# fractalclockwork/CS267_HW3

Measured on NVIDIA B200. Metric: kmers_per_s_insert_plus_traverse, higher is better.
Workload: dtype u128

## Files before the change

cs267_hw3_b200/csrc/ctable.cuh:

```cuda
#pragma once
#include "kernels.cuh"

namespace kh {

#ifndef KH_CT_BUCKETS2
#define KH_CT_BUCKETS2 2176
#endif
#ifndef KH_CT_THREADS
#define KH_CT_THREADS 512
#endif
#ifndef KH_CT_MINBLOCKS
#define KH_CT_MINBLOCKS 2
#endif
#ifndef KH_CT_JUMPS
#define KH_CT_JUMPS 3
#endif
template <int W> struct CtBuild {
    static constexpr u32 kMaxBuckets = (W == 1) ? 1536u : (u32)KH_CT_BUCKETS2;
    static constexpr u32 kMaxSlots = kMaxBuckets * (u32)Slot<W>::kPerBucket;
    static constexpr u32 kOffSucc = kMaxBuckets * 32u;
    static constexpr u32 kOffPd = kOffSucc + kMaxSlots * 2u;
    static constexpr u32 kOffOff = kOffPd + kMaxSlots * 4u;
    static constexpr u32 kOffCode = kOffOff + kMaxSlots * 2u;
    static constexpr u32 kSmem = kOffCode + kMaxSlots;
// ... 280 lines not shown
    }
}

__global__ void ct_mark_filed_kernel(const u32* __restrict__ xin_cnt, u32* __restrict__ xin_done, const u32* __restrict__ extra_cnt,
                                     u32* __restrict__ extra_done, const CtCaps caps, int world) {
    const int s = (int)threadIdx.x;
    if (s < world) xin_done[s] = min(xin_cnt[s], caps.xin_cap);
    if (s == 0) *extra_done = min(*extra_cnt, caps.extra_cap);
}

__global__ void __launch_bounds__(1024)
ct_layout_kernel(const u32* __restrict__ chunk_cursor, u32 nchunks, const CtGeom g, const CtCaps caps, u32 per_bucket, u32 max_slots,
                 u32* __restrict__ chunk_base, u32* __restrict__ pool_off, Counters* ctr) {
    __shared__ u64 s_warp[33];
    constexpr u32 kPer = 8;
    u64 carry_b = 0, carry_p = 0;
    for (u32 c0 = 0; c0 < nchunks; c0 += blockDim.x * kPer) {
        const u32 first = c0 + threadIdx.x * kPer;
        u32 capb[kPer], chars[kPer];
        u64 sum_b = 0, sum_p = 0;
#pragma unroll
        for (u32 q = 0; q < kPer; ++q) {
            const u32 c = first + q;
            capb[q] = 0; chars[q] = 0;
            if (c < nchunks) {
                const u32 load = min(chunk_cursor[c], max_slots);
                if (load) {
                    const u64 want_slots = ((u64)load * g.lf_inv_q16 + 65535u) >> 16;
                    capb[q] = (u32)min((u64)g.max_buckets, max((want_slots + per_bucket - 1) / per_bucket, (u64)(load / per_bucket + 1)));
                }
                chars[q] = (load + 15u) & ~15u;
            }
            sum_b += capb[q]; sum_p += chars[q];
        }
        u64 tot_b, tot_p;
        u64 eb = carry_b + block_exclusive_scan(sum_b, s_warp, tot_b);
        u64 ep = carry_p + block_exclusive_scan(sum_p, s_warp, tot_p);
#pragma unroll
        for (u32 q = 0; q < kPer; ++q) {
            const u32 c = first + q;
            if (c < nchunks) { chunk_base[c] = (u32)eb; pool_off[c] = (u32)ep; }
            eb += capb[q]; ep += chars[q];
        }
        carry_b += tot_b; carry_p += tot_p;
    }
    if (threadIdx.x == 0) {
        chunk_base[nchunks] = (u32)carry_b;
        pool_off[nchunks] = (u32)carry_p;
        if (carry_b > caps.nbuckets_alloc || carry_p > caps.pool_cap) atomicOr(&ctr->errors, kErrTableFull);
    }
}

template <int W> __device__ __forceinline__ u32 ct_tag(typename Slot<W>::value_t v);
template <> __device__ __forceinline__ u32 ct_tag<1>(u64 v) { return (u32)(v >> 6); }
template <> __device__ __forceinline__ u32 ct_tag<2>(u128 v) { return (u32)(v.lo >> 6); }

template <int W, bool VOLATILE>
__device__ __forceinline__ void ct_lds_tags(unsigned saddr, u64 (&w)[4]) {
    if (W == 1) {
        if (VOLATILE) {
            asm volatile("ld.volatile.shared.v2.u64 {%0,%1}, [%2];" : "=l"(w[0]), "=l"(w[1]) : "r"(saddr) : "memory");
            asm volatile("ld.volatile.shared.v2.u64 {%0,%1}, [%2+16];" : "=l"(w[2]), "=l"(w[3]) : "r"(saddr) : "memory");
        } else {
            asm volatile("ld.shared.v2.u64 {%0,%1}, [%2];" : "=l"(w[0]), "=l"(w[1]) : "r"(saddr));
            asm volatile("ld.shared.v2.u64 {%0,%1}, [%2+16];" : "=l"(w[2]), "=l"(w[3]) : "r"(saddr));
        }
    } else {
        if (VOLATILE) {
            asm volatile("ld.volatile.shared.u64 %0, [%1];" : "=l"(w[0]) : "r"(saddr) : "memory");
            asm volatile("ld.volatile.shared.u64 %0, [%1+16];" : "=l"(w[1]) : "r"(saddr) : "memory");
        } else {
            asm volatile("ld.shared.u64 %0, [%1];" : "=l"(w[0]) : "r"(saddr));
            asm volatile("ld.shared.u64 %0, [%1+16];" : "=l"(w[1]) : "r"(saddr));
        }
    }
}
__device__ __forceinline__ u64 ct_lds64(unsigned saddr) {
    u64 x;
    asm volatile("ld.volatile.shared.u64 %0, [%1];" : "=l"(x) : "r"(saddr) : "memory");
    return x;
}
template <int W> __device__ __forceinline__ bool ct_verify(unsigned saddr, int i, u64 low, typename Slot<W>::value_t key, u64& idx_word);
template <> __device__ __forceinline__ bool ct_verify<1>(unsigned, int, u64 low, u64 key, u64& idx_word) {
    idx_word = low;
    return CtSlot<1>::same_key(low, key);
}
template <> __device__ __forceinline__ bool ct_verify<2>(unsigned saddr, int i, u64 low, u128 key, u64& idx_word) {
    idx_word = ct_lds64(saddr + 16u * i + 8u);
    return (((idx_word ^ key.hi) << kIdxBits) | ((low ^ key.lo) >> 6)) == 0ull;
}

template <int W>
__device__ __forceinline__ int ct_smem_insert(typename Slot<W>::value_t* s_tab, unsigned s_base, u32 nb, typename Slot<W>::value_t val) {
    typedef Slot<W> S;
    typedef typename S::value_t V;
    const u32 tag = ct_tag<W>(val);
    u32 b = ct_bucket_in_chunk(CtSlot<W>::hash32(val), nb);
    for (u32 tries = 0; tries < nb;) {
        u64 w[4];
        ct_lds_tags<W, true>(s_base + b * 32u, w);
        int j = -1;
        u32 match = 0;
#pragma unroll
        for (int i = S::kPerBucket - 1; i >= 0; --i) {
            const bool e = ((u32)w[i] & 7u) == 0u;
            j = e ? i : j;
            match |= (!e && (u32)(w[i] >> 6) == tag) ? (1u << i) : 0u;
        }
        if (match) {
#pragma unroll
            for (int i = 0; i < S::kPerBucket; ++i) {
                u64 iw;
                if ((match >> i) & 1u) if (ct_verify<W>(s_base + b * 32u, i, w[i], val, iw)) return -1;
            }
        }
        if (j < 0) { b = (b + 1 == nb) ? 0u : b + 1; ++tries; continue; }
        const V old = S::cas_shared(s_tab + b * S::kPerBucket + j, S::zero(), val);
        if (S::empty(old)) return (int)(b * S::kPerBucket + j);
        if (CtSlot<W>::same_key(old, val)) return -1;
    }
    return -2;
}

constexpr int kFindMiss = -1, kFindNext = -2;
template <int W>
__device__ __forceinline__ void ct_lds_bucket(unsigned saddr, u64 (&q)[4]) {
    asm volatile("ld.shared.v2.u64 {%0,%1}, [%2];" : "=l"(q[0]), "=l"(q[1]) : "r"(saddr));
    asm volatile("ld.shared.v2.u64 {%0,%1}, [%2+16];" : "=l"(q[2]), "=l"(q[3]) : "r"(saddr));
}
template <int W> __device__ __forceinline__ int ct_find_step(unsigned saddr, typename Slot<W>::value_t key);
template <> __device__ __forceinline__ int ct_find_step<1>(unsigned saddr, u64 key) {
    u64 q[4];
    ct_lds_bucket<1>(saddr, q);
    int res = kFindNext;
#pragma unroll
    for (int i = 3; i >= 0; --i) {
        const bool e = ((u32)q[i] & 7u) == 0u;
        const bool m = (((q[i] ^ key) << kIdxBits) >> (kIdxBits + 6)) == 0ull;
        res = e ? kFindMiss : (m ? (int)(q[i] >> (64 - kIdxBits)) - 1 : res);
    }
    return res;
}
template <> __device__ __forceinline__ int ct_find_step<2>(unsigned saddr, u128 key) {
    u64 q[4];
    ct_lds_bucket<2>(saddr, q);
    int res = kFindNext;
#pragma unroll
    for (int i = 1; i >= 0; --i) {
        const bool e = ((u32)q[2 * i] & 7u) == 0u;
        const bool m = (((q[2 * i + 1] ^ key.hi) << kIdxBits) | ((q[2 * i] ^ key.lo) >> 6)) == 0ull;
        res = e ? kFindMiss : (m ? (int)(q[2 * i + 1] >> (64 - kIdxBits)) - 1 : res);
    }
    return res;
}

template <int W>
__global__ void __launch_bounds__(kCtBuildThreads, KH_CT_MINBLOCKS)
ct_build_kernel(const typename Slot<W>::value_t* __restrict__ fine, const u32* __restrict__ chunk_cursor,
                const u32* __restrict__ chunk_base, const u32* __restrict__ pool_off,
                typename Slot<W>::value_t* __restrict__ table, u32* __restrict__ seg_base,
                u64* __restrict__ link, u64* __restrict__ meta, typename Slot<W>::value_t* __restrict__ ext_key,
                unsigned char* __restrict__ pool, const CtGeom g, const CtCaps caps, Counters* ctr) {
    typedef Slot<W> S;
    typedef CtSlot<W> CS;
    typedef typename S::value_t V;
    typedef CtBuild<W> B;
    extern __shared__ __align__(128) unsigned char s_bld[];
    unsigned char* const s_raw = s_bld;
    V* s_tab = reinterpret_cast<V*>(s_raw);
    unsigned short* s_succ = reinterpret_cast<unsigned short*>(s_raw + B::kOffSucc);
    unsigned char* s_pool = s_raw + B::kOffSucc;
    u32* s_pd = reinterpret_cast<u32*>(s_raw + B::kOffPd);
    unsigned short* s_off = reinterpret_cast<unsigned short*>(s_raw + B::kOffOff);
    unsigned char* s_code = s_raw + B::kOffCode;
    __shared__ u32 s_inserted, s_dups, s_nheads, s_seg0, s_chars, s_err;
    const u32 c = blockIdx.x;
    const u32 b0 = chunk_base[c], nb = chunk_base[c + 1] - b0;
    const u32 cnt = min(chunk_cursor[c], B::kMaxSlots);
    if (nb == 0) {
        if (threadIdx.x == 0) seg_base[c] = 0;
        return;
    }
    const unsigned s_base = (unsigned)__cvta_generic_to_shared(s_tab);
    const int k = g.k;
    constexpr int kBatch = 4;
    V v[kBatch];
#pragma unroll
    for (int r = 0; r < kBatch; ++r) {
        const u32 i = threadIdx.x + r * kCtBuildThreads;
        v[r] = i < cnt ? fine[ct_fine_index<W>(c, i, g.chunks_per_rank)] : S::zero();
    }
    if (threadIdx.x == 0) { s_inserted = 0; s_dups = 0; s_nheads = 0; s_chars = 0; s_err = 0; }
    {
        uint4* s4 = reinterpret_cast<uint4*>(s_raw);
        for (u32 i = threadIdx.x; i < nb * 2u; i += kCtBuildThreads) s4[i] = make_uint4(0, 0, 0, 0);
        for (u32 i = threadIdx.x; i < cnt; i += kCtBuildThreads) s_pd[i] = (kPredNone << 16) | 1u;
    }
    __syncthreads();
    u32 inserted = 0, dups = 0, err = 0;
    for (u32 base = 0; base < cnt; base += kCtBuildThreads * kBatch) {
        V nxt[kBatch];
#pragma unroll
        for (int r = 0; r < kBatch; ++r) {
            const u32 i = base + kCtBuildThreads * kBatch + threadIdx.x + r * kCtBuildThreads;
            nxt[r] = i < cnt ? fine[ct_fine_index<W>(c, i, g.chunks_per_rank)] : S::zero();
        }
#pragma unroll
        for (int r = 0; r < kBatch; ++r) {
            const u32 node = base + threadIdx.x + r * kCtBuildThreads;
            if (node >= cnt) continue;
            const int slot = ct_smem_insert<W>(s_tab, s_base, nb, CS::with_idx(v[r], node + 1u));
            inserted += (slot >= 0);
            dups += (slot == -1);
            if (slot == -2) err |= kErrTableFull;
            s_succ[node] = (unsigned short)(slot >= 0 ? (u32)slot : kSuccDead);
        }
#pragma unroll
        for (int r = 0; r < kBatch; ++r) v[r] = nxt[r];
    }
    inserted = __reduce_add_sync(kFullMask, inserted);
    dups = __reduce_add_sync(kFullMask, dups);
    err = __reduce_or_sync(kFullMask, err);
    if (lane_id() == 0) {
        if (inserted) atomicAdd(&s_inserted, inserted);
        if (dups) atomicAdd(&s_dups, dups);
        if (err) atomicOr(&s_err, err);
    }
    __syncthreads();
#pragma unroll 1
    for (u32 base = threadIdx.x; base < cnt; base += 2 * kCtBuildThreads) {
        u32 slot[2], b[2], code[2];
        V key[2];
        int res[2];
#pragma unroll
        for (int q = 0; q < 2; ++q) {
            const u32 node = base + q * kCtBuildThreads;
            slot[q] = node < cnt ? (u32)s_succ[node] : kSuccDead;
        }
#pragma unroll
        for (int q = 0; q < 2; ++q) {
            const V cur = slot[q] != kSuccDead ? s_tab[slot[q]] : S::zero();
            const u32 f = slot[q] != kSuccDead ? S::fwd(cur) : kExtF;
            code[q] = f | ((slot[q] != kSuccDead && S::back(cur) == kExtF) ? kCodeBackF : 0u);
            key[q] = S::next_key(CS::strip(cur), k);
            b[q] = ct_bucket_in_chunk(CS::hash32(key[q]), nb);
        }
#pragma unroll
        for (int q = 0; q < 2; ++q) res[q] = (code[q] & 7u) != kExtF ? ct_find_step<W>(s_base + b[q] * 32u, key[q]) : kFindMiss;
#pragma unroll
        for (int q = 0; q < 2; ++q) {
            for (u32 tries = 1; res[q] == kFindNext && tries < nb; ++tries) {
                b[q] = (b[q] + 1 == nb) ? 0u : b[q] + 1;
                res[q] = ct_find_step<W>(s_base + b[q] * 32u, key[q]);
            }
        }
#pragma unroll
        for (int q = 0; q < 2; ++q) {
            const u32 node = base + q * kCtBuildThreads;
            if (node >= cnt) continue;
            s_code[node] = (unsigned char)code[q];
            u32 sc = slot[q] == kSuccDead ? kSuccDead : kSuccTail;
            if ((code[q] & 7u) != kExtF) {
                if (res[q] < 0) {
                    sc = kSuccExt | slot[q];
                } else {
                    sc = (u32)res[q];
                    s_pd[res[q]] = (node << 16) | 1u;
                }
            }
            s_succ[node] = (unsigned short)sc;
        }
    }
    __syncthreads();
#pragma unroll 1
    for (u32 node = threadIdx.x; node < cnt; node += kCtBuildThreads) {
        const u32 s = s_succ[node];
        if (s < kSuccExt && (s_pd[s] >> 16) != node) s_code[s] |= (unsigned char)kCodeMulti;
    }
    __syncthreads();
    for (u32 base = 0; base < cnt; base += kCtBuildThreads) {
        const u32 node = base + threadIdx.x;
        bool head = false, dead = true;
        if (node < cnt) {
            dead = s_succ[node] == kSuccDead;
            head = !dead && ((s_pd[node] >> 16) == kPredNone || (s_code[node] & (kCodeBackF | kCodeMulti)));
        }
        const u32 bal = __ballot_sync(kFullMask, head);
        u32 first = 0;
        if (lane_id() == 0 && bal) first = atomicAdd(&s_nheads, (u32)__popc(bal));
        first = __shfl_sync(kFullMask, first, 0);
        if (head) s_pd[node] = (node << 16) | (first + __popc(bal & ((1u << lane_id()) - 1u)));
        else if (dead && node < cnt) s_pd[node] = node << 16;
    }
    __syncthreads();
    const u32 nheads = s_nheads;
    if (threadIdx.x == 0) {
        u32 seg0 = nheads ? atomicAdd(&ctr->next_seg, nheads) : 0u;
        if (seg0 + nheads > caps.seg_cap) { ct_internal(ctr, kSiteSegCap); seg0 = caps.seg_cap; }
        s_seg0 = seg0;
        seg_base[c] = seg0;
    }
    u32 active = 0;
#pragma unroll 1
    for (u32 i = 0, node = threadIdx.x; node < cnt; ++i, node += kCtBuildThreads) {
        const u32 pd = s_pd[node];
        active |= ((pd >> 16) != node) ? (1u << i) : 0u;
    }
    for (int round = 0; round < (14 + KH_CT_JUMPS - 1) / KH_CT_JUMPS; ++round) {
#pragma unroll 1
        for (int rep = 0; rep < KH_CT_JUMPS; ++rep) {
#pragma unroll 1
            for (u32 m = active; m; m &= m - 1u) {
                const u32 i = (u32)__ffs((int)m) - 1u, node = threadIdx.x + i * kCtBuildThreads;
                const u32 pd = s_pd[node], a = pd >> 16;
                const u32 pa = s_pd[a], a2 = pa >> 16;
                if (a2 == a) { active &= ~(1u << i); continue; }
                s_pd[node] = (a2 << 16) | ((pd + pa) & 0xFFFFu);
            }
        }
        if (!__syncthreads_or(active != 0u)) break;
    }
    __syncthreads();
    const u32 seg0 = s_seg0;
    const u32 my_bits = (u32)g.rank << kRankShift;
    const u64 pool0 = pool_off[c];
    if (seg0 < caps.seg_cap) {
    #pragma unroll 1
    for (u32 node = threadIdx.x; node < cnt; node += kCtBuildThreads) {
            const u32 s = s_succ[node];
            if (s == kSuccDead) continue;
            const u32 pd = s_pd[node], a = pd >> 16;
            const bool root = a == node;
            const u32 pa = root ? pd : s_pd[a];
            if ((pa >> 16) != a) continue;
            const u32 f = s_code[node] & 7u;
            bool last = f == kExtF || s >= kSuccExt;
            u32 next_hi = f == kExtF ? kLinkTail : kLinkPending;
            if (!last) {
                const u32 ps = s_pd[s];
                if ((ps >> 16) == s) { last = true; next_hi = my_bits | (seg0 + (ps & 0xFFFFu)); }
            }
            if (!last) continue;
            const u32 n = (root ? 0u : (pd & 0xFFFFu)) + (f != kExtF ? 1u : 0u);
            const u32 off = atomicAdd(&s_chars, n);
            s_off[a] = (unsigned short)off;
            const u32 gseg = seg0 + (pa & 0xFFFFu);
            link[gseg] = ((u64)next_hi << 32) | (next_hi == kLinkTail ? 0u : n);
            meta[gseg] = ((pool0 + off) << 24) | n;
            if (next_hi == kLinkPending) ext_key[gseg] = S::next_key(CS::strip(s_tab[s & 0x7FFFu]), k);
        }
    }
    __syncthreads();
#pragma unroll 1
    for (u32 node = threadIdx.x; node < cnt; node += kCtBuildThreads) {
        const u32 code = s_code[node];
        if ((code & 7u) == kExtF) continue;
        const u32 pd = s_pd[node], a = pd >> 16;
        const bool root = a == node;
        if (!root && (s_pd[a] >> 16) != a) continue;
        s_pool[(u32)s_off[a] + (root ? 0u : (pd & 0xFFFFu))] = ext_char(code & 7u);
    }
    {
        const u32 nslots = nb * S::kPerBucket;
        for (u32 i = threadIdx.x; i < nslots; i += kCtBuildThreads) {
            const V cur = s_tab[i];
            if (S::empty(cur)) continue;
            const u32 node = CS::idx(cur) - 1u, pd = s_pd[node];
            s_tab[i] = CS::with_idx(cur, (pd >> 16) == node ? (pd & 0xFFFFu) + 1u : 0u);
        }
    }
    asm volatile("fence.proxy.async.shared::cta;" ::: "memory");
    __syncthreads();
    {
        const u32 tab_bytes = nb * 32u, pool_bytes = (s_chars + 15u) & ~15u;
        constexpr u32 kPiece = 8192u;
        const u32 tab_pieces = (tab_bytes + kPiece - 1u) / kPiece, pool_pieces = (pool_bytes + kPiece - 1u) / kPiece;
        if (lane_id() == 0) {
            unsigned char* g_tab = reinterpret_cast<unsigned char*>(table + (u64)b0 * S::kPerBucket);
            bool any = false;
            for (u32 pc = threadIdx.x >> 5; pc < tab_pieces + pool_pieces; pc += kCtBuildThreads / 32) {
                const bool is_tab = pc < tab_pieces;
                const u32 o = (is_tab ? pc : pc - tab_pieces) * kPiece;
                const u32 bytes = min(kPiece, (is_tab ? tab_bytes : pool_bytes) - o);
                const unsigned src = (unsigned)__cvta_generic_to_shared(is_tab ? s_raw + o : s_pool + o);
                unsigned char* dst = is_tab ? g_tab + o : pool + pool0 + o;
                asm volatile("cp.async.bulk.global.shared::cta.bulk_group [%0], [%1], %2;" ::"l"(dst), "r"(src), "r"(bytes) : "memory");
                any = true;
            }
            if (any) {
                asm volatile("cp.async.bulk.commit_group;" ::: "memory");
                asm volatile("cp.async.bulk.wait_group.read 0;" ::: "memory");
            }
        }
    }
    if (threadIdx.x == 0) {
        if (s_inserted) atomicAdd(&ctr->n_inserted, (u64)s_inserted);
        if (s_dups) atomicAdd(&ctr->n_duplicates, (u64)s_dups);
        if (s_err) atomicOr(&ctr->errors, s_err);
    }
}

template <int W>
__device__ __forceinline__ bool ct_lookup_chunk(const typename Slot<W>::value_t* __restrict__ table, const u32* __restrict__ chunk_base,
                                                u32 chunk, typename Slot<W>::value_t key, typename Slot<W>::value_t& found) {
    typedef Slot<W> S;
    typedef typename S::value_t V;
    const u32 b0 = chunk_base[chunk], nb = chunk_base[chunk + 1] - b0;
    if (nb == 0) return false;
    u32 b = ct_bucket_in_chunk(CtSlot<W>::hash32(key), nb);
    for (u32 tries = 0; tries < nb; ++tries) {
        u64 q[4];
        load256_nc(table + (u64)(b0 + b) * S::kPerBucket, q);
        bool hole = false, hit = false;
#pragma unroll
        for (int i = 0; i < S::kPerBucket; ++i) {
            const V cur = S::from_bucket(q, i);
            const bool e = S::empty(cur);
            if (!hole && !hit && !e && CtSlot<W>::same_key(cur, key)) { found = cur; hit = true; }
            hole = hole || e;
        }
        if (hit) return true;
        if (hole) return false;
        b = (b + 1 == nb) ? 0u : b + 1;
    }
    return false;
}
// ... 445 lines not shown
```

cs267_hw3_b200/csrc/slot.cuh:

```cuda
#pragma once
#include <cstdint>
#include <cuda_runtime.h>

namespace kh {

typedef unsigned long long u64;
typedef unsigned int u32;

constexpr u32 kExtF = 4;
constexpr u32 kExtBad = 7;

struct alignas(16) u128 {
    u64 lo, hi;
};

constexpr u64 ext_lut_entry(u64 lut, int idx, u64 code) { return (lut & ~(7ull << (3 * idx))) | (code << (3 * idx)); }
constexpr u64 kExtLut = ext_lut_entry(ext_lut_entry(ext_lut_entry(ext_lut_entry(ext_lut_entry(
                            0x7FFFFFFFFFFFFFFFull, 1, 0), 3, 1), 6, 4), 7, 2), 20, 3);
__host__ __device__ __forceinline__ u32 ext_code(unsigned char c) {
    const u32 i = c & 31u;
    const bool letter = (c & 0xE0u) == 0x40u && i <= 20u;
    return letter ? ((u32)(kExtLut >> (3u * i)) & 7u) : kExtBad;
}
#ifdef __CUDACC__
// ... 246 lines not shown


__host__ __device__ __forceinline__ int minimizer_len(int k) {
    return k <= 14 ? k : (k <= 18 ? 11 : (k <= 29 ? 13 : (k <= 40 ? 21 : 31)));
}
__host__ __device__ __forceinline__ u32 mmer_order(u64 x) {
    return (u32)((x * 0x9E3779B97F4A7C15ull) >> 32);
}
template <int W> __host__ __device__ __forceinline__ u64 minimizer_value(typename Slot<W>::value_t v, int k, int m);
template <> __host__ __device__ __forceinline__ u64 minimizer_value<1>(u64 v, int k, int m) {
    const u64 key = v >> 6, mask = (m >= 32) ? ~0ull : ((1ull << (2 * m)) - 1ull);
    u32 best = 0xFFFFFFFFu;
    u64 bx = 0;
    for (int s = 2 * (k - m); s >= 0; s -= 2) {
        const u64 x = (key >> s) & mask;
        const u32 g = mmer_order(x);
        if (g < best) { best = g; bx = x; }
    }
    return bx;
}
template <> __host__ __device__ __forceinline__ u64 minimizer_value<2>(u128 v, int k, int m) {
    const u64 lo = (v.lo >> 6) | (v.hi << 58), hi = v.hi >> 6, mask = (m >= 32) ? ~0ull : ((1ull << (2 * m)) - 1ull);
    u32 best = 0xFFFFFFFFu;
    u64 bx = 0;
    for (int s = 2 * (k - m); s >= 0; s -= 2) {
        const u64 x = (s >= 64 ? (hi >> (s - 64)) : (s == 0 ? lo : ((lo >> s) | (hi << (64 - s))))) & mask;
        const u32 g = mmer_order(x);
        if (g < best) { best = g; bx = x; }
    }
    return bx;
}
__host__ __device__ __forceinline__ int owner_minimizer_len(int k) { return k <= 14 ? k : 7; }

template <int W> __host__ __device__ __forceinline__ u64 owner_hash_of(typename Slot<W>::value_t v, int k, int m) {
    return m ? fmix64(minimizer_value<W>(v, k, m) + 0x632BE59BD9B4E019ull) : Slot<W>::owner_hash(v);
}

__host__ __device__ __forceinline__ u64 bucket_of(u64 h, u64 nbuckets) {
#ifdef __CUDA_ARCH__
    return __umul64hi(h, nbuckets);
#else
    return (u64)(((unsigned __int128)h * nbuckets) >> 64);
#endif
}

template <int W>
__host__ __device__ __forceinline__ u32 owner_of(typename Slot<W>::value_t v, int world, int k, int m) {
    return (u32)bucket_of(owner_hash_of<W>(v, k, m), (u64)world);
}

template <int W> struct RegionOf { static constexpr u64 kBuckets = (W == 1) ? 4 : 16; };
template <int W>
__host__ __device__ __forceinline__ u64 place_bucket_from(u64 minimizer_hash, typename Slot<W>::value_t v, u64 nbuckets) {
    constexpr u64 G = RegionOf<W>::kBuckets;
    const u64 region = bucket_of(fmix64(minimizer_hash ^ 0x9E3779B97F4A7C15ull), nbuckets / G);
    return region * G + (Slot<W>::hash(v) & (G - 1));
}
template <int W>
__host__ __device__ __forceinline__ u64 place_bucket(typename Slot<W>::value_t v, int k, int m, u64 nbuckets) {
    if (m == 0) return bucket_of(Slot<W>::hash(v), nbuckets);
    return place_bucket_from<W>(fmix64(minimizer_value<W>(v, k, m) + 0x632BE59BD9B4E019ull), v, nbuckets);
}

constexpr u32 kIdxBits = 14;
constexpr u32 kMinMul = 0x9E3779B1u;
constexpr u32 kMinAdd = 0x7F4A7C15u;

__host__ __device__ __forceinline__ int ct_minimizer_len(int k) { return k >= 31 ? 15 : (k >= 23 ? 13 : (k >= 17 ? k - 6 : k)); }
__host__ __device__ __forceinline__ int ct_window(int k) { const int w = k - ct_minimizer_len(k) + 1; return w > 32 ? 32 : w; }
__host__ __device__ __forceinline__ bool ct_supported(int k) { return k >= 17 && k <= 54; }
__host__ __device__ __forceinline__ int ct_slot_words(int k) { return (2 * k + 6 + (int)kIdxBits <= 64) ? 1 : 2; }

__host__ __device__ __forceinline__ u32 ct_funnel_r(u32 lo, u32 hi, u32 s) {
#ifdef __CUDA_ARCH__
    return __funnelshift_r(lo, hi, s);
#else
    return s ? ((lo >> s) | (hi << (32 - s))) : lo;
#endif
}
__host__ __device__ __forceinline__ u32 ct_mulhi32(u32 a, u32 b) {
#ifdef __CUDA_ARCH__
    return __umulhi(a, b);
#else
    return (u32)(((u64)a * b) >> 32);
#endif
}
__host__ __device__ __forceinline__ u32 ct_min_hash_words(u32 a, u32 b, u32 c, u32 d, int m, int win) {
    const u32 mul = kMinMul << (32 - 2 * m);
    u32 best = 0xFFFFFFFFu;
    int rem = win;
    for (int it = 0; it < 2; ++it) {
        if (rem >= 16) {
#pragma unroll
            for (int j = 0; j < 16; ++j) {
                const u32 h = ct_funnel_r(a, b, 2u * j) * mul + kMinAdd;
                best = h < best ? h : best;
            }
        } else {
#pragma unroll
            for (int j = 0; j < 16; ++j) {
                u32 h = ct_funnel_r(a, b, 2u * j) * mul + kMinAdd;
                h = (j < rem) ? h : 0xFFFFFFFFu;
                best = h < best ? h : best;
            }
        }
        if (rem <= 16) break;
        rem -= 16; a = b; b = c; c = d; d = 0;
    }
    return best;
}
template <int W> __host__ __device__ __forceinline__ u32 ct_min_hash(typename Slot<W>::value_t v, int m, int win);
template <> __host__ __device__ __forceinline__ u32 ct_min_hash<1>(u64 v, int m, int win) {
    const u64 key = v >> 6;
    return ct_min_hash_words((u32)key, (u32)(key >> 32), 0u, 0u, m, win);
}
template <> __host__ __device__ __forceinline__ u32 ct_min_hash<2>(u128 v, int m, int win) {
    const u64 lo = (v.lo >> 6) | (v.hi << 58), hi = v.hi >> 6;
    return ct_min_hash_words((u32)lo, (u32)(lo >> 32), (u32)hi, (u32)(hi >> 32), m, win);
}

__host__ __device__ __forceinline__ u32 ct_fmix32_hi(u32 h) {
    h ^= h >> 15; h *= 0x85EBCA6Bu;
    h ^= h >> 13; h *= 0xC2B2AE35u;
    return h;
}
template <int W> struct CtSlot;
template <> struct CtSlot<1> {
    typedef u64 V;
    static __host__ __device__ __forceinline__ V strip(V v) { return v & (~0ull >> kIdxBits); }
    static __host__ __device__ __forceinline__ u32 idx(V v) { return (u32)(v >> (64 - kIdxBits)); }
    static __host__ __device__ __forceinline__ V with_idx(V v, u32 i) { return strip(v) | ((u64)i << (64 - kIdxBits)); }
    static __host__ __device__ __forceinline__ bool same_key(V a, V b) { return (((a ^ b) << kIdxBits) >> (kIdxBits + 6)) == 0ull; }
    static __host__ __device__ __forceinline__ u32 hash32(V v) {
        const u32 x0 = (u32)v & ~63u, x1 = (u32)(v >> 32) & (0xFFFFFFFFu >> kIdxBits);
        return ct_fmix32_hi((x0 * 0x9E3779B1u) ^ x1);
    }
};
template <> struct CtSlot<2> {
    typedef u128 V;
    static __host__ __device__ __forceinline__ V strip(V v) { return u128{v.lo, v.hi & (~0ull >> kIdxBits)}; }
    static __host__ __device__ __forceinline__ u32 idx(V v) { return (u32)(v.hi >> (64 - kIdxBits)); }
    static __host__ __device__ __forceinline__ V with_idx(V v, u32 i) { return u128{v.lo, (v.hi & (~0ull >> kIdxBits)) | ((u64)i << (64 - kIdxBits))}; }
    static __host__ __device__ __forceinline__ bool same_key(V a, V b) { return (((a.hi ^ b.hi) << kIdxBits) | ((a.lo ^ b.lo) >> 6)) == 0ull; }
    static __host__ __device__ __forceinline__ u32 hash32(V v) {
        const u32 x0 = (u32)v.lo & ~63u, x1 = (u32)(v.lo >> 32), x2 = (u32)v.hi, x3 = (u32)(v.hi >> 32) & (0xFFFFFFFFu >> kIdxBits);
        u32 h = x0 * 0x9E3779B1u;
        h = (h ^ x1) * 0x85EBCA77u;
        h = (h ^ x2) * 0xC2B2AE3Du;
        return ct_fmix32_hi(h ^ x3);
    }
};
__host__ __device__ __forceinline__ u32 ct_bucket_in_chunk(u32 h32, u32 nb) { return ct_mulhi32(h32, nb); }

struct CtGeom {
    int k, m, win;
    int world, rank;
    u32 chunks_per_rank;
    u32 max_buckets;
    u32 lf_inv_q16;
};
__host__ __device__ __forceinline__ void ct_place(u32 minhash, const CtGeom& g, u32& owner, u32& chunk) {
    const u32 u = ct_fmix32_hi(minhash ^ (minhash >> 16));
    owner = ct_mulhi32(u, (u32)g.world);
    chunk = ct_mulhi32(u, (u32)g.world * g.chunks_per_rank) - owner * g.chunks_per_rank;
}

constexpr int kMaxRanks = 8;
constexpr u32 kRankShift = 28;
constexpr u32 kLocalMask = (1u << kRankShift) - 1u;
constexpr u32 kLinkFinalBit = 0x80000000u;
constexpr u32 kLinkDistMask = 0x7FFFFFFFu;
constexpr u32 kLinkMissing = 0xFFFFFFFBu;
constexpr u32 kLinkConverge = 0xFFFFFFFAu;
constexpr u32 kLinkLoop = kLinkConverge;
constexpr u32 kLinkCtFirstMarker = kLinkConverge;

enum : u32 {
    kErrNotFound = 1u, kErrTableFull = 2u, kErrCycle = 4u, kErrBadInput = 8u,
    kErrConverge = 16u, kErrInternal = 32u
};

constexpr u32 kLinkTail = 0xFFFFFFFFu;
constexpr u32 kLinkUnused = 0xFFFFFFFEu;
constexpr u32 kLinkClaimed = 0xFFFFFFFDu;
constexpr u32 kLinkPending = 0xFFFFFFFCu;
constexpr u32 kLinkFirstMarker = kLinkPending;

enum : u32 { kSiteBarrier = 1u, kSiteStarts = 2u, kSiteSegCap = 4u, kSiteInbox = 8u, kSiteStubOpen = 16u, kSiteOutCap = 32u };

struct Counters {
    u32 next_walker;
    u32 next_seg;
    u32 errors;
    u32 rank_rounds;
    u64 n_inserted;
    u64 n_duplicates;
    u64 scan_total;
    u64 n_nodes;
    u64 contig_bytes;
    u32 n_boundary;
    u32 n_outbox;
    u32 flags[40];
    u32 rank_done;
    u32 err_where;
    u64 n_starts_dev;
    u32 need_jump;
    u32 use_jump;
};

}
```

Baseline: 12.59 billion.

## Build chunk hash table by counting-sort run placement instead of probed atomic inserts

```diff
diff --git a/cs267_hw3_b200/csrc/ctable.cuh b/cs267_hw3_b200/csrc/ctable.cuh
--- a/cs267_hw3_b200/csrc/ctable.cuh
+++ b/cs267_hw3_b200/csrc/ctable.cuh
@@ -456,6 +456,143 @@
         res = e ? kFindMiss : (m ? (int)(q[2 * i + 1] >> (64 - kIdxBits)) - 1 : res);
     }
     return res;
+}
+
+template <int kPerBucket>
+__device__ __forceinline__ void ct_run_directory(const u32* s_cnt, u32* s_dir, u32 nb, u32 nslots, int* s_part) {
+    constexpr int kNone = -0x40000000;
+    constexpr int kWarps = kCtBuildThreads / 32;
+    const u32 per = (nb + kCtBuildThreads - 1) / kCtBuildThreads;
+    const u32 h0 = min(nb, threadIdx.x * per), h1 = min(nb, h0 + per);
+    int s = 0, d = kNone;
+    for (u32 h = h0; h < h1; ++h) { d = max(d, kPerBucket * (int)h - s); s += (int)s_cnt[h]; }
+    const int lane = (int)lane_id(), warp = (int)(threadIdx.x >> 5);
+#pragma unroll
+    for (int o = 1; o < 32; o <<= 1) {
+        const int ps = __shfl_up_sync(kFullMask, s, o), pd = __shfl_up_sync(kFullMask, d, o);
+        if (lane >= o) { d = max(pd, d - ps); s += ps; }
+    }
+    if (lane == 31) { s_part[2 * warp] = s; s_part[2 * warp + 1] = d; }
+    int es = __shfl_up_sync(kFullMask, s, 1), ed = __shfl_up_sync(kFullMask, d, 1);
+    if (lane == 0) { es = 0; ed = kNone; }
+    __syncthreads();
+    int ws = 0, wd = kNone, ts = 0, td = kNone;
+#pragma unroll
+    for (int w = 0; w < kWarps; ++w) {
+        if (w == warp) { ws = ts; wd = td; }
+        td = max(td, s_part[2 * w + 1] - ts);
+        ts += s_part[2 * w];
+    }
+    const u32 carry = ct_run_carry((u32)ts, (u32)max(td, 0), nslots);
+    int S = ws + es, D = max(wd, ed - ws);
+    for (u32 h = h0; h < h1; ++h) {
+        D = max(D, kPerBucket * (int)h - S);
+        const u32 n = s_cnt[h];
+        s_dir[h] = (ct_run_slot(ct_run_start((u32)S, (u32)D, carry), 0u, nslots) << 16) | n;
+        S += (int)n;
+    }
+}
+
+template <int W>
+__device__ __forceinline__ void ct_build_probed(const typename Slot<W>::value_t* __restrict__ fine, u32 c, u32 cnt, u32 nb, int k, u32 chunks_per_rank,
+                                             unsigned char* s_raw, u32* s_inserted, u32* s_dups, u32* s_err) {
+    typedef Slot<W> S;
+    typedef CtSlot<W> CS;
+    typedef typename S::value_t V;
+    typedef CtBuild<W> B;
+    V* s_tab = reinterpret_cast<V*>(s_raw);
+    unsigned short* s_succ = reinterpret_cast<unsigned short*>(s_raw + B::kOffSucc);
+    u32* s_pd = reinterpret_cast<u32*>(s_raw + B::kOffPd);
+    unsigned char* s_code = s_raw + B::kOffCode;
+    const unsigned s_base = (unsigned)__cvta_generic_to_shared(s_tab);
+    constexpr int kBatch = 4;
+    V v[kBatch];
+#pragma unroll
+    for (int r = 0; r < kBatch; ++r) {
+        const u32 i = threadIdx.x + r * kCtBuildThreads;
+        v[r] = i < cnt ? fine[ct_fine_index<W>(c, i, chunks_per_rank)] : S::zero();
+    }
+    {
+        uint4* s4 = reinterpret_cast<uint4*>(s_raw);
+        for (u32 i = threadIdx.x; i < nb * 2u; i += kCtBuildThreads) s4[i] = make_uint4(0, 0, 0, 0);
+        for (u32 i = threadIdx.x; i < cnt; i += kCtBuildThreads) s_pd[i] = (kPredNone << 16) | 1u;
+    }
+    __syncthreads();
+    u32 inserted = 0, dups = 0, err = 0;
+    for (u32 base = 0; base < cnt; base += kCtBuildThreads * kBatch) {
+        V nxt[kBatch];
+#pragma unroll
+        for (int r = 0; r < kBatch; ++r) {
+            const u32 i = base + kCtBuildThreads * kBatch + threadIdx.x + r * kCtBuildThreads;
+            nxt[r] = i < cnt ? fine[ct_fine_index<W>(c, i, chunks_per_rank)] : S::zero();
+        }
+#pragma unroll
+        for (int r = 0; r < kBatch; ++r) {
+            const u32 node = base + threadIdx.x + r * kCtBuildThreads;
+            if (node >= cnt) continue;
+            const int slot = ct_smem_insert<W>(s_tab, s_base, nb, CS::with_idx(v[r], node + 1u));
+            inserted += (slot >= 0);
+            dups += (slot == -1);
+            if (slot == -2) err |= kErrTableFull;
+            s_succ[node] = (unsigned short)(slot >= 0 ? (u32)slot : kSuccDead);
+        }
+#pragma unroll
+        for (int r = 0; r < kBatch; ++r) v[r] = nxt[r];
+    }
+    inserted = __reduce_add_sync(kFullMask, inserted);
+    dups = __reduce_add_sync(kFullMask, dups);
+    err = __reduce_or_sync(kFullMask, err);
+    if (lane_id() == 0) {
+        if (inserted) atomicAdd(s_inserted, inserted);
+        if (dups) atomicAdd(s_dups, dups);
+        if (err) atomicOr(s_err, err);
+    }
+    __syncthreads();
+#pragma unroll 1
+    for (u32 base = threadIdx.x; base < cnt; base += 2 * kCtBuildThreads) {
+        u32 slot[2], b[2], code[2];
+        V key[2];
+        int res[2];
+#pragma unroll
+        for (int q = 0; q < 2; ++q) {
+            const u32 node = base + q * kCtBuildThreads;
+            slot[q] = node < cnt ? (u32)s_succ[node] : kSuccDead;
+        }
+#pragma unroll
+        for (int q = 0; q < 2; ++q) {
+            const V cur = slot[q] != kSuccDead ? s_tab[slot[q]] : S::zero();
+            const u32 f = slot[q] != kSuccDead ? S::fwd(cur) : kExtF;
+            code[q] = f | ((slot[q] != kSuccDead && S::back(cur) == kExtF) ? kCodeBackF : 0u);
+            key[q] = S::next_key(CS::strip(cur), k);
+            b[q] = ct_bucket_in_chunk(CS::hash32(key[q]), nb);
+        }
+#pragma unroll
+        for (int q = 0; q < 2; ++q) res[q] = (code[q] & 7u) != kExtF ? ct_find_step<W>(s_base + b[q] * 32u, key[q]) : kFindMiss;
+#pragma unroll
+        for (int q = 0; q < 2; ++q) {
+            for (u32 tries = 1; res[q] == kFindNext && tries < nb; ++tries) {
+                b[q] = (b[q] + 1 == nb) ? 0u : b[q] + 1;
+                res[q] = ct_find_step<W>(s_base + b[q] * 32u, key[q]);
+            }
+        }
+#pragma unroll
+        for (int q = 0; q < 2; ++q) {
+            const u32 node = base + q * kCtBuildThreads;
+            if (node >= cnt) continue;
+            s_code[node] = (unsigned char)code[q];
+            u32 sc = slot[q] == kSuccDead ? kSuccDead : kSuccTail;
+            if ((code[q] & 7u) != kExtF) {
+                if (res[q] < 0) {
+                    sc = kSuccExt | slot[q];
+                } else {
+                    sc = (u32)res[q];
+                    s_pd[res[q]] = (node << 16) | 1u;
+                }
+            }
+            s_succ[node] = (unsigned short)sc;
+        }
+    }
+    __syncthreads();
 }
 
 template <int W>
@@ -487,95 +624,117 @@
     }
     const unsigned s_base = (unsigned)__cvta_generic_to_shared(s_tab);
     const int k = g.k;
+    const u32 nslots = nb * S::kPerBucket;
     constexpr int kBatch = 4;
-    V v[kBatch];
-#pragma unroll
-    for (int r = 0; r < kBatch; ++r) {
-        const u32 i = threadIdx.x + r * kCtBuildThreads;
-        v[r] = i < cnt ? fine[ct_fine_index<W>(c, i, g.chunks_per_rank)] : S::zero();
-    }
     if (threadIdx.x == 0) { s_inserted = 0; s_dups = 0; s_nheads = 0; s_chars = 0; s_err = 0; }
-    {
-        uint4* s4 = reinterpret_cast<uint4*>(s_raw);
-        for (u32 i = threadIdx.x; i < nb * 2u; i += kCtBuildThreads) s4[i] = make_uint4(0, 0, 0, 0);
-        for (u32 i = threadIdx.x; i < cnt; i += kCtBuildThreads) s_pd[i] = (kPredNone << 16) | 1u;
-    }
-    __syncthreads();
-    u32 inserted = 0, dups = 0, err = 0;
-    for (u32 base = 0; base < cnt; base += kCtBuildThreads * kBatch) {
-        V nxt[kBatch];
+    bool built = false;
+    if (cnt <= nslots) {
+        u32* s_cnt = s_pd;
+        u32* s_dir = reinterpret_cast<u32*>(s_off);
+        V v[kBatch];
 #pragma unroll
         for (int r = 0; r < kBatch; ++r) {
-            const u32 i = base + kCtBuildThreads * kBatch + threadIdx.x + r * kCtBuildThreads;
-            nxt[r] = i < cnt ? fine[ct_fine_index<W>(c, i, g.chunks_per_rank)] : S::zero();
-        }
-#pragma unroll
-        for (int r = 0; r < kBatch; ++r) {
-            const u32 node = base + threadIdx.x + r * kCtBuildThreads;
-            if (node >= cnt) continue;
-            const int slot = ct_smem_insert<W>(s_tab, s_base, nb, CS::with_idx(v[r], node + 1u));
-            inserted += (slot >= 0);
-            dups += (slot == -1);
-            if (slot == -2) err |= kErrTableFull;
-            s_succ[node] = (unsigned short)(slot >= 0 ? (u32)slot : kSuccDead);
-        }
-#pragma unroll
-        for (int r = 0; r < kBatch; ++r) v[r] = nxt[r];
-    }
-    inserted = __reduce_add_sync(kFullMask, inserted);
-    dups = __reduce_add_sync(kFullMask, dups);
-    err = __reduce_or_sync(kFullMask, err);
-    if (lane_id() == 0) {
-        if (inserted) atomicAdd(&s_inserted, inserted);
-        if (dups) atomicAdd(&s_dups, dups);
-        if (err) atomicOr(&s_err, err);
-    }
-    __syncthreads();
+            const u32 i = threadIdx.x + r * kCtBuildThreads;
+            v[r] = i < cnt ? fine[ct_fine_index<W>(c, i, g.chunks_per_rank)] : S::zero();
+        }
+        {
+            uint4* s4 = reinterpret_cast<uint4*>(s_raw);
+            for (u32 i = threadIdx.x; i < nb * 2u; i += kCtBuildThreads) s4[i] = make_uint4(0, 0, 0, 0);
+            for (u32 i = threadIdx.x; i < nb; i += kCtBuildThreads) s_cnt[i] = 0;
+        }
+        __syncthreads();
+        for (u32 base = 0; base < cnt; base += kCtBuildThreads * kBatch) {
+#pragma unroll
+            for (int r = 0; r < kBatch; ++r) {
+                const u32 node = base + threadIdx.x + r * kCtBuildThreads;
+                if (node >= cnt) continue;
+                const V x = base == 0 ? v[r] : fine[ct_fine_index<W>(c, node, g.chunks_per_rank)];
+                s_succ[node] = (unsigned short)atomicAdd(&s_cnt[ct_bucket_in_chunk(CS::hash32(x), nb)], 1u);
+            }
+        }
+        __syncthreads();
+        ct_run_directory<S::kPerBucket>(s_cnt, s_dir, nb, nslots, reinterpret_cast<int*>(s_code));
+        __syncthreads();
+        for (u32 base = 0; base < cnt; base += kCtBuildThreads * kBatch) {
+#pragma unroll
+            for (int r = 0; r < kBatch; ++r) {
+                const u32 node = base + threadIdx.x + r * kCtBuildThreads;
+                if (node >= cnt) continue;
+                const V x = base == 0 ? v[r] : fine[ct_fine_index<W>(c, node, g.chunks_per_rank)];
+                const u32 slot = ct_run_slot(s_dir[ct_bucket_in_chunk(CS::hash32(x), nb)] >> 16, s_succ[node], nslots);
+                s_tab[slot] = CS::with_idx(x, node + 1u);
+                s_succ[node] = (unsigned short)slot;
+                s_pd[node] = (kPredNone << 16) | 1u;
+            }
+        }
+        __syncthreads();
+        const u64* s_lo = reinterpret_cast<const u64*>(s_tab);
+        bool dup = false;
 #pragma unroll 1
-    for (u32 base = threadIdx.x; base < cnt; base += 2 * kCtBuildThreads) {
-        u32 slot[2], b[2], code[2];
-        V key[2];
-        int res[2];
-#pragma unroll
-        for (int q = 0; q < 2; ++q) {
-            const u32 node = base + q * kCtBuildThreads;
-            slot[q] = node < cnt ? (u32)s_succ[node] : kSuccDead;
-        }
-#pragma unroll
-        for (int q = 0; q < 2; ++q) {
-            const V cur = slot[q] != kSuccDead ? s_tab[slot[q]] : S::zero();
-            const u32 f = slot[q] != kSuccDead ? S::fwd(cur) : kExtF;
-            code[q] = f | ((slot[q] != kSuccDead && S::back(cur) == kExtF) ? kCodeBackF : 0u);
-            key[q] = S::next_key(CS::strip(cur), k);
-            b[q] = ct_bucket_in_chunk(CS::hash32(key[q]), nb);
-        }
-#pragma unroll
-        for (int q = 0; q < 2; ++q) res[q] = (code[q] & 7u) != kExtF ? ct_find_step<W>(s_base + b[q] * 32u, key[q]) : kFindMiss;
-#pragma unroll
-        for (int q = 0; q < 2; ++q) {
-            for (u32 tries = 1; res[q] == kFindNext && tries < nb; ++tries) {
-                b[q] = (b[q] + 1 == nb) ? 0u : b[q] + 1;
-                res[q] = ct_find_step<W>(s_base + b[q] * 32u, key[q]);
-            }
-        }
-#pragma unroll
-        for (int q = 0; q < 2; ++q) {
-            const u32 node = base + q * kCtBuildThreads;
-            if (node >= cnt) continue;
-            s_code[node] = (unsigned char)code[q];
-            u32 sc = slot[q] == kSuccDead ? kSuccDead : kSuccTail;
-            if ((code[q] & 7u) != kExtF) {
-                if (res[q] < 0) {
-                    sc = kSuccExt | slot[q];
-                } else {
-                    sc = (u32)res[q];
-                    s_pd[res[q]] = (node << 16) | 1u;
+        for (u32 base = threadIdx.x; base < cnt; base += 2 * kCtBuildThreads) {
+            u32 slot[2], code[2], pos[2], left[2];
+            V key[2];
+            int res[2];
+#pragma unroll
+            for (int q = 0; q < 2; ++q) {
+                const u32 node = base + q * kCtBuildThreads;
+                slot[q] = node < cnt ? (u32)s_succ[node] : kSuccDead;
+                const V cur = slot[q] != kSuccDead ? s_tab[slot[q]] : S::zero();
+                const u32 f = slot[q] != kSuccDead ? S::fwd(cur) : kExtF;
+                code[q] = f | ((slot[q] != kSuccDead && S::back(cur) == kExtF) ? kCodeBackF : 0u);
+                key[q] = S::next_key(CS::strip(cur), k);
+                const u32 d = s_dir[ct_bucket_in_chunk(CS::hash32(key[q]), nb)];
+                pos[q] = d >> 16;
+                left[q] = (code[q] & 7u) != kExtF ? (d & 0xFFFFu) : 0u;
+                res[q] = kFindMiss;
+                if (slot[q] != kSuccDead) {
+                    const u32 tag = ct_tag<W>(cur);
+                    for (u32 p = s_dir[ct_bucket_in_chunk(CS::hash32(cur), nb)] >> 16; p != slot[q]; p = (p + 1 == nslots) ? 0u : p + 1) {
+                        const u64 lo = s_lo[p * W];
+                        u64 iw;
+                        if ((u32)(lo >> 6) == tag && ct_verify<W>(s_base + p * (u32)sizeof(V), 0, lo, cur, iw)) dup = true;
+                    }
                 }
             }
-            s_succ[node] = (unsigned short)sc;
-        }
-    }
-    __syncthreads();
+            while ((left[0] | left[1]) != 0u) {
+#pragma unroll
+                for (int q = 0; q < 2; ++q) {
+                    if (!left[q]) continue;
+                    const u64 lo = s_lo[pos[q] * W];
+                    u64 iw;
+                    if ((u32)(lo >> 6) == ct_tag<W>(key[q]) && ct_verify<W>(s_base + pos[q] * (u32)sizeof(V), 0, lo, key[q], iw)) {
+                        res[q] = (int)(iw >> (64 - kIdxBits)) - 1;
+                        left[q] = 0;
+                    } else {
+                        --left[q];
+                        pos[q] = (pos[q] + 1 == nslots) ? 0u : pos[q] + 1;
+                    }
+                }
+            }
+#pragma unroll
+            for (int q = 0; q < 2; ++q) {
+                const u32 node = base + q * kCtBuildThreads;
+                if (node >= cnt) continue;
+                s_code[node] = (unsigned char)code[q];
+                u32 sc = kSuccTail;
+                if ((code[q] & 7u) != kExtF) {
+                    if (res[q] < 0) {
+                        sc = kSuccExt | slot[q];
+                    } else {
+                        sc = (u32)res[q];
+                        s_pd[res[q]] = (node << 16) | 1u;
+                    }
+                }
+                s_succ[node] = (unsigned short)sc;
+            }
+        }
+        built = !__syncthreads_or(dup);
+    }
+    if (built) {
+        if (threadIdx.x == 0) s_inserted = cnt;
+    } else {
+        ct_build_probed<W>(fine, c, cnt, nb, k, g.chunks_per_rank, s_raw, &s_inserted, &s_dups, &s_err);
+    }
 #pragma unroll 1
     for (u32 node = threadIdx.x; node < cnt; node += kCtBuildThreads) {
         const u32 s = s_succ[node];
diff --git a/cs267_hw3_b200/csrc/slot.cuh b/cs267_hw3_b200/csrc/slot.cuh
--- a/cs267_hw3_b200/csrc/slot.cuh
+++ b/cs267_hw3_b200/csrc/slot.cuh
@@ -422,6 +422,16 @@
 };
 __host__ __device__ __forceinline__ u32 ct_bucket_in_chunk(u32 h32, u32 nb) { return ct_mulhi32(h32, nb); }
 
+__host__ __device__ __forceinline__ u32 ct_run_carry(u32 total, u32 d_last, u32 nslots) {
+    const u32 end = total + d_last;
+    return end > nslots ? end - nslots : 0u;
+}
+__host__ __device__ __forceinline__ u32 ct_run_start(u32 s, u32 d, u32 carry) { return s + (d > carry ? d : carry); }
+__host__ __device__ __forceinline__ u32 ct_run_slot(u32 start, u32 rank, u32 nslots) {
+    const u32 p = start + rank;
+    return p >= nslots ? p - nslots : p;
+}
+
 struct CtGeom {
     int k, m, win;
     int world, rank;
```

Result: faster. 12.84 billion (median of 6 runs) (+2.0%).
